# Gancheekim/ATM-VFI

Measured on AMD Instinct MI355X. Metric: interpolated frames/s at 1080p (network_base, bs=1), higher is better.
Workload: dtype f32 (contractions as fp16 hi/lo split x3 MFMA, fp32 accumulate; ~22 significand bits)

## Files before the change

### atm-vfi_amd/csrc/gemm_common.h

```cpp
#pragma once
#include "common.h"

namespace atmvfi {

struct GemmDev {
    int mode;
    const float* in;
    int in_ld, H, W, Cin;
    long long in_gstride;
    int in_rpg;
    const float* weight;
    int wrows;
    int ktot;
    int cin_pad;
    int cpt;
    int nchunks;
    int Cout;
    int coutp;
    int kw, stride, pad, dil;
    int Ho, Wo;
    long long M;
    float* out;
    int out_ld;
    long long out_gstride;
    int out_rpg;
    const int* out_row_map;
    const float* bias;
    const float* prelu;
    const float* in_prelu;
    const float* residual;
    int res_ld;
    const _Float16* w_hi;
    const _Float16* w_lo;
    int cin_pad32;
    int cpt32;
    int nchunks32;
    int ktot32;
    const _Float16* a_hi;
    const _Float16* a_lo;
    const _Float16* a_hi2;
    const _Float16* a_lo2;
    int in_ld2, split_chunks;
    int in_N;
    unsigned long long* stamp;
    int dbg;
    int mchunk;
    int vblocks;
    int nblocks;
    _Float16* out_hi;
    _Float16* out_lo;
    long long out_plane_rows;
    int out_c0, out_gc;
    int force_wn;
    int ksplit;
    float* part;
    long long part_stride;
    int part_ld;
    int fit32;
    int pfit32;
};


__device__ __forceinline__ bool gemm_out_row(const GemmDev& a, long long m, float*& orow, const float*& rrow, long long& prow, int& pc0) {
    pc0 = a.out_c0;
    if (a.mode == ATMVFI_GEMM_DECONV) {
        const int hw = a.H * a.W;
        const int n = (m >> 31) ? (int)(m / hw) : (int)((unsigned)m / (unsigned)hw);
        const int rem = (int)(m - (long long)n * hw);
        const int y = rem / a.W;
        const int x = rem - y * a.W;
        prow = ((long long)n * a.Ho + 2 * y) * a.Wo + 2 * x;
        orow = a.out + prow * a.out_ld;
    } else {
        long long ro = m;
        if (a.out_row_map) ro = a.out_row_map[m];
        if (ro < 0) return false;
        prow = ro;
        long long off = ro * (long long)a.out_ld;
        if (a.out_rpg > 0) {
            const long long grp = ro / a.out_rpg;
            prow = ro - grp * a.out_rpg;
            off = grp * a.out_gstride + prow * (long long)a.out_ld;
            pc0 += (int)grp * a.out_gc;
        }
        orow = a.out + off;
    }
    rrow = a.residual ? a.residual + m * (long long)a.res_ld : nullptr;
    return true;
}
__device__ __forceinline__ void gemm_out_row_at(const GemmDev& a, long long m, long long ro, float*& orow, long long& prow, int& pc0) {
    pc0 = a.out_c0;
    if (a.mode == ATMVFI_GEMM_DECONV) {
        const int hw = a.H * a.W;
        const int n = (m >> 31) ? (int)(m / hw) : (int)((unsigned)m / (unsigned)hw);
        const int rem = (int)(m - (long long)n * hw);
        const int y = rem / a.W;
        const int x = rem - y * a.W;
        prow = ((long long)n * a.Ho + 2 * y) * a.Wo + 2 * x;
        orow = a.out + prow * a.out_ld;
    } else {
        prow = ro;
        long long off = ro * (long long)a.out_ld;
        if (a.out_rpg > 0) {
            const long long grp = ro / a.out_rpg;
            prow = ro - grp * a.out_rpg;
            off = grp * a.out_gstride + prow * (long long)a.out_ld;
            pc0 += (int)grp * a.out_gc;
        }
        orow = a.out + off;
    }
}
__device__ __forceinline__ bool gemm_out_row(const GemmDev& a, long long m, float*& orow, const float*& rrow) {
    long long prow;
    int pc0;
    return gemm_out_row(a, m, orow, rrow, prow, pc0);
}

struct ChanVec {
    f32x4 b, p;
    int co;
    int q;
    int nvalid;
};

__device__ __forceinline__ ChanVec gemm_chan_vec(const GemmDev& a, int nb) {
    ChanVec c;
    c.q = 0;
    c.co = nb;
    if (a.mode == ATMVFI_GEMM_DECONV) {
        c.q = (nb >= a.coutp) + (nb >= 2 * a.coutp) + (nb >= 3 * a.coutp);
        c.co = nb - c.q * a.coutp;
        if (nb >= 4 * a.coutp) c.co = -1;
    }
    if (c.co >= a.Cout) c.co = -1;
    c.nvalid = c.co < 0 ? 0 : a.Cout - c.co;
    c.b = (f32x4){0.f, 0.f, 0.f, 0.f};
    c.p = (f32x4){1.f, 1.f, 1.f, 1.f};
    if (c.nvalid >= 4) {
        if (a.bias) c.b = *reinterpret_cast<const f32x4*>(a.bias + c.co);
        if (a.prelu) c.p = *reinterpret_cast<const f32x4*>(a.prelu + c.co);
    } else if (c.nvalid > 0) {
        float bb[4] = {0.f, 0.f, 0.f, 0.f}, pp[4] = {1.f, 1.f, 1.f, 1.f};
// ... 108 lines not shown
```

### atm-vfi_amd/csrc/gemm_conv.hip

```cpp
#include "common.h"
#include "gemm_common.h"

#include <algorithm>

namespace {

using atmvfi::GemmDev;

__device__ __forceinline__ int swz(int row) { return (0x1320 >> (((row >> 2) & 3) << 2)) & 3; }

template <int WM, int WN>
__global__ __launch_bounds__(256) void gemm_mfma_f32(const GemmDev a) {
    fp16_saturate_on();
    constexpr int BM = 64 * WM;
    constexpr int BN = 16 * WN;
    constexpr int NB = (BN * 4 + 255) / 256;
    __shared__ __attribute__((aligned(16))) float lds[2 * (BM + BN) * 16];
    float* As = lds;
    float* Bs = lds + 2 * BM * 16;

    const int t = threadIdx.x;
    const int lane = t & 63;
    const int wave = t >> 6;
    const int kq = t & 3;
// ... 230 lines not shown
                           "gemm: a second plane source needs CONV mode, both planes, in_ld2 > N*H*W and 0 < 32 * in_split_chunks < Cin");
        }
    }
    ATMVFI_REQUIRE(p->mode >= 0 && p->mode <= 2, ATMVFI_EINVAL, "gemm: bad mode %d", p->mode);
    ATMVFI_REQUIRE(p->Cin > 0 && p->Cout > 0, ATMVFI_EINVAL, "gemm: bad channel counts");
    ATMVFI_REQUIRE(planes || (p->in_ld >= atmvfi::round_up(p->Cin, 4) && p->in_ld % 4 == 0), ATMVFI_EALIGN,
                   "gemm: in_ld %d must be a multiple of 4 and >= Cin rounded to 4 (Cin %d)", p->in_ld, p->Cin);
    ATMVFI_REQUIRE(!p->out || (p->out_ld % 4 == 0 && p->out_ld >= atmvfi::round_up(p->Cout, 4)), ATMVFI_EALIGN,
                   "gemm: out_ld %d must be a multiple of 4 and >= Cout rounded to 4 (Cout %d)", p->out_ld, p->Cout);
    ATMVFI_REQUIRE((planes || atmvfi::aligned16(p->in)) && (!p->out || atmvfi::aligned16(p->out)) && atmvfi::aligned16(p->weight), ATMVFI_EALIGN,
                   "gemm: in/out/weight must be 16-byte aligned");
    ATMVFI_REQUIRE((planes || p->in_gstride % 4 == 0) && p->out_gstride % 4 == 0, ATMVFI_EALIGN, "gemm: group strides must be multiples of 4");
    if (p->residual)
        ATMVFI_REQUIRE(p->res_ld >= p->Cout, ATMVFI_EINVAL, "gemm: res_ld %d < Cout %d", p->res_ld, p->Cout);
    if (p->in_prelu) ATMVFI_REQUIRE(atmvfi::aligned16(p->in_prelu), ATMVFI_EALIGN, "gemm: in_prelu must be 16-byte aligned");
    ATMVFI_REQUIRE((!p->bias || atmvfi::aligned16(p->bias)) && (!p->prelu || atmvfi::aligned16(p->prelu)) &&
                       (!p->residual || (atmvfi::aligned16(p->residual) && p->res_ld % 4 == 0)),
                   ATMVFI_EALIGN, "gemm: bias/prelu/residual must be 16-byte aligned (res_ld a multiple of 4)");

    GemmDev d;
    d.mode = p->mode;
    d.in = p->in; d.in_ld = p->in_ld; d.H = p->H; d.W = p->W; d.Cin = p->Cin;
    d.in_gstride = p->in_gstride; d.in_rpg = p->in_rpg;
    d.weight = p->weight;
    d.cin_pad = atmvfi::round_up(p->Cin, 16);
    d.cpt = d.cin_pad / 16;
    d.Cout = p->Cout; d.coutp = atmvfi::round_up(p->Cout, 4);
    d.kw = 1; d.stride = 1; d.pad = 0; d.dil = 1; d.Ho = p->Ho; d.Wo = p->Wo;
    int taps = 1;
    int ngemm = p->Cout;
    if (p->mode == ATMVFI_GEMM_CONV) {
        ATMVFI_REQUIRE(p->N > 0 && p->H > 0 && p->W > 0, ATMVFI_EINVAL, "conv2d: bad input size");
        ATMVFI_REQUIRE((p->kh == 1 || p->kh == 3) && p->kh == p->kw, ATMVFI_EINVAL, "conv2d: kernel %dx%d unsupported", p->kh, p->kw);
        ATMVFI_REQUIRE(p->stride >= 1 && p->dil >= 1 && p->pad >= 0, ATMVFI_EINVAL, "conv2d: bad stride/dilation/pad");
        const int ho = (p->H + 2 * p->pad - p->dil * (p->kh - 1) - 1) / p->stride + 1;
        const int wo = (p->W + 2 * p->pad - p->dil * (p->kw - 1) - 1) / p->stride + 1;
        ATMVFI_REQUIRE(ho == p->Ho && wo == p->Wo, ATMVFI_EINVAL, "conv2d: Ho/Wo (%d,%d) do not match geometry (%d,%d)", p->Ho, p->Wo, ho, wo);
        ATMVFI_REQUIRE(p->in_rpg == 0 && p->out_rpg == 0 && !p->out_row_map, ATMVFI_EINVAL, "conv2d: row groups/maps are LINEAR-only");
        taps = p->kh * p->kw;
        d.kw = p->kw; d.stride = p->stride; d.pad = p->pad; d.dil = p->dil;
        d.M = (long long)p->N * p->Ho * p->Wo;
        ATMVFI_REQUIRE(p->M == 0 || p->M == d.M, ATMVFI_EINVAL, "conv2d: M mismatch");
    } else if (p->mode == ATMVFI_GEMM_LINEAR) {
        ATMVFI_REQUIRE(p->M > 0, ATMVFI_EINVAL, "linear: M must be > 0");
        d.H = 1; d.W = 1;
        d.M = p->M;
    } else {
        ATMVFI_REQUIRE(p->N > 0 && p->H > 0 && p->W > 0, ATMVFI_EINVAL, "deconv: bad input size");
        ATMVFI_REQUIRE(p->Ho == 2 * p->H && p->Wo == 2 * p->W, ATMVFI_EINVAL, "deconv: Ho/Wo must be 2H/2W");
        ATMVFI_REQUIRE(p->in_rpg == 0 && p->out_rpg == 0 && !p->out_row_map && !p->residual, ATMVFI_EINVAL, "deconv: unsupported option");
        d.M = (long long)p->N * p->H * p->W;
        ngemm = 4 * d.coutp;
    }
    d.wrows = packed_rows(p->mode, p->Cout);
    d.ktot = taps * d.cin_pad;
    d.nchunks = taps * d.cpt;
    d.out = p->out; d.out_ld = p->out_ld; d.out_gstride = p->out_gstride; d.out_rpg = p->out_rpg;
    d.out_row_map = p->out_row_map;
    d.bias = p->bias; d.prelu = p->prelu; d.in_prelu = p->in_prelu; d.residual = p->residual; d.res_ld = p->res_ld;
    ATMVFI_REQUIRE(d.M < (1ll << 40), ATMVFI_EINVAL, "gemm: M too large");
    d.a_hi = (const _Float16*)p->in_hi;
    d.a_lo = (const _Float16*)p->in_lo;
    d.a_hi2 = (const _Float16*)p->in_hi2;
    d.a_lo2 = (const _Float16*)p->in_lo2;
    d.in_ld2 = p->in_ld2;
    d.split_chunks = p->in_hi2 ? p->in_split_chunks : (1 << 30);
    d.in_N = p->N;
    d.out_hi = (_Float16*)p->out_hi;
    d.out_lo = (_Float16*)p->out_lo;
    d.out_plane_rows = p->out_plane_rows;
    d.out_c0 = p->out_plane_c0;
    d.out_gc = p->out_plane_gc;
    ATMVFI_REQUIRE(p->tile_wn >= -4 && p->tile_wn <= 8 && (p->tile_wn >= 0 || planes), ATMVFI_EINVAL,
                   "gemm: tile_wn 0 (auto), 1..8, or (split-plane input) -1 reference schedule / -2 gemm_duo (128-column tiles) / -3 gemm_pp / -4 gemm_duo (64-column tiles), got %d", p->tile_wn);
    d.force_wn = p->tile_wn;
    ATMVFI_REQUIRE(!p->workspace || (atmvfi::aligned16(p->workspace) && p->workspace_floats > 0), ATMVFI_EALIGN,
                   "gemm: the split-K workspace must be 16-byte aligned and non-empty");
    d.ksplit = 0;
    d.part = p->workspace;
    d.part_stride = p->workspace ? p->workspace_floats : 0;
    d.part_ld = 0;
    d.fit32 = 0;
    d.pfit32 = 0;
    d.nblocks = 0;
    d.dbg = 0;
    d.vblocks = 0;
    d.mchunk = 0;
    d.stamp = nullptr;
    d.w_hi = (const _Float16*)p->weight_hi;
    d.w_lo = (const _Float16*)p->weight_lo;
    d.cin_pad32 = atmvfi::round_up(p->Cin, 32);
    d.cpt32 = d.cin_pad32 / 32;
    d.nchunks32 = taps * d.cpt32;
    d.ktot32 = taps * d.cin_pad32;
    if (p->precision == ATMVFI_PREC_F16X3) {
        ATMVFI_REQUIRE(p->weight_hi && p->weight_lo, ATMVFI_EINVAL, "gemm: precision f16x3 needs weight_hi/weight_lo");
        ATMVFI_REQUIRE(atmvfi::aligned16(p->weight_hi) && atmvfi::aligned16(p->weight_lo), ATMVFI_EALIGN,
                       "gemm: split weights must be 16-byte aligned");
        if (planes) return atmvfi::launch_gemm_split(d, ngemm, (hipStream_t)stream);
        return atmvfi::launch_gemm_f16x3(d, ngemm, (hipStream_t)stream);
    }

    {
        int rc = 0;
        if (atmvfi::try_launch_conv3x3_small(d, p->kh, &rc, (hipStream_t)stream)) return rc;
    }
    const int ntiles = (ngemm + 15) / 16;
    int best = 1;
    float best_cost = 1e30f;
    for (int wn = 1; wn <= 8; ++wn) {
        const int padded = (ntiles + wn - 1) / wn * wn;
        const float cost = (float)padded * (1.0f + 1.0f / (float)wn);
        if (cost <= best_cost) { best_cost = cost; best = wn; }
    }
    hipStream_t s = (hipStream_t)stream;
    switch (best) {
        case 1: launch<2, 1>(d, ntiles, s); break;
        case 2: launch<2, 2>(d, ntiles, s); break;
        case 3: launch<2, 3>(d, ntiles, s); break;
        case 4: launch<2, 4>(d, ntiles, s); break;
        case 5: launch<2, 5>(d, ntiles, s); break;
        case 6: launch<2, 6>(d, ntiles, s); break;
        case 7: launch<2, 7>(d, ntiles, s); break;
        default: launch<2, 8>(d, ntiles, s); break;
    }
    return atmvfi::check_launch("gemm");
}

extern "C" int atmvfi_conv2d(const atmvfi_gemm_params* p, void* stream) {
    ATMVFI_REQUIRE(p && p->mode == ATMVFI_GEMM_CONV, ATMVFI_EINVAL, "conv2d: params->mode must be ATMVFI_GEMM_CONV");
    return atmvfi_gemm(p, stream);
}
extern "C" int atmvfi_linear(const atmvfi_gemm_params* p, void* stream) {
    ATMVFI_REQUIRE(p && p->mode == ATMVFI_GEMM_LINEAR, ATMVFI_EINVAL, "linear: params->mode must be ATMVFI_GEMM_LINEAR");
    return atmvfi_gemm(p, stream);
}
extern "C" int atmvfi_deconv2x2(const atmvfi_gemm_params* p, void* stream) {
    ATMVFI_REQUIRE(p && p->mode == ATMVFI_GEMM_DECONV, ATMVFI_EINVAL, "deconv2x2: params->mode must be ATMVFI_GEMM_DECONV");
    return atmvfi_gemm(p, stream);
}
```

### atm-vfi_amd/csrc/gemm_duo.hip

```cpp
#include "gemm_plane.h"

namespace {

using atmvfi::GemmDev;

constexpr int BM = 128;
constexpr int stage_bytes(int BN) { return (2 * BM + 2 * BN) * 64; }
constexpr int A_LO = BM * 64, W_HI = 2 * BM * 64;
constexpr int cst_floats(int BN) { return atmvfi::gemm_const_floats(BN) + BM; }

#ifdef ATMVFI_STAMP
static unsigned long long* g_duo_stamp = nullptr;
extern "C" void atmvfi_debug_set_duo_stamp_buffer(void* p) { g_duo_stamp = (unsigned long long*)p; }
#define DUO_SUB(k) do { if (a.stamp) { __builtin_amdgcn_sched_barrier(0); const unsigned long long t_ = __builtin_amdgcn_s_memtime(); sub[k] += t_ - sub_t; sub_t = t_; __builtin_amdgcn_sched_barrier(0); } } while (0)
#else
#define DUO_SUB(k) do { } while (0)
#endif

template <bool CONVM, int BN>
__global__ __launch_bounds__(256, 2) void gemm_duo_kernel(const GemmDev a) {
    constexpr int STAGE = stage_bytes(BN), W_LO = W_HI + BN * 64;
    constexpr int MI = BN == 128 ? 4 : 2;
    constexpr int NWN = BN / 64;
    constexpr int WROWS = 16 * MI;
// ... 71 lines not shown
            dma16(pa_lo + aoff[1], dst + A_LO + 4 * 1024);
            pa_hi += a_step;
            pa_lo += a_step;
        }
        dma16(pw_hi + wsoff[0], dst + W_HI);
        if constexpr (PIW == 2) dma16(pw_hi + wsoff[1], dst + W_HI + 4 * 1024);
        dma16(pw_lo + wsoff[0], dst + W_LO);
        if constexpr (PIW == 2) dma16(pw_lo + wsoff[1], dst + W_LO + 4 * 1024);
        pw_hi += w_step;
        pw_lo += w_step;
    };
    {
        atmvfi::gemm_dma_consts<BN>(a, n0, cst_w, wave, lane);
        if (a.out_row_map && a.mode == ATMVFI_GEMM_LINEAR) {
            int m = m0 + (wave & 1) * 64 + lane;
            if (m >= M) m = M - 1;
            __builtin_amdgcn_global_load_lds((const __attribute__((address_space(1))) void*)(a.out_row_map + m),
                                             (__attribute__((address_space(3))) void*)(cst_w + atmvfi::gemm_const_floats(BN) + (wave & 1) * 64), 4, 0, 0);
        } else {
            atmvfi::gemm_dma_consts<BN>(a, n0, cst_w, wave, lane);
        }
    }

    f32x4 acc[MI][4], cor[MI][4];
#pragma unroll
    for (int i = 0; i < MI; ++i)
#pragma unroll
        for (int j = 0; j < 4; ++j) {
            acc[i][j] = (f32x4){0.f, 0.f, 0.f, 0.f};
            cor[i][j] = (f32x4){0.f, 0.f, 0.f, 0.f};
        }
#ifdef ATMVFI_STAMP
    unsigned long long sub[8] = {0, 0, 0, 0, 0, 0, 0, 0}, sub_t = 0, t_begin = 0;
    if (a.stamp) { t_begin = sub_t = __builtin_amdgcn_s_memtime(); }
#endif
    issue_stage(0);
    if (nk > 1) issue_stage(1);
    DUO_SUB(0);
    f16x8 xh[MI], xl[MI], wh[4], wl[4];
    const unsigned xfrag = lds_offset(smem) + (unsigned)((WROWS * wm + r) * 64 + ((g ^ swz64(r)) << 4));
    const unsigned wfrag = lds_offset(smem) + (unsigned)(W_HI + (64 * wn + r) * 64 + ((g ^ swz64(r)) << 4));
    for (int u = 0; u < nk; ++u) {
        if (u + 1 < nk) wait_vm<4 + 2 * PIW>();
        else wait_vm<0>();
        __builtin_amdgcn_s_barrier();
        DUO_SUB(1);
        const unsigned off = (unsigned)((u & 1) * STAGE);
        static_for<0, MI>([&](auto ic) {
            constexpr int i = decltype(ic)::value;
            lds_read16<i * 1024>(xh[i], xfrag + off);
            lds_read16<i * 1024 + A_LO>(xl[i], xfrag + off);
        });
        static_for<0, 4>([&](auto jc) {
            constexpr int j = decltype(jc)::value;
            lds_read16<j * 1024>(wh[j], wfrag + off);
            lds_read16<j * 1024 + BN * 64>(wl[j], wfrag + off);
        });
        asm volatile("s_waitcnt lgkmcnt(0)" : "+v"(xh[0]), "+v"(xh[1]), "+v"(xl[0]), "+v"(xl[1]));
        if constexpr (MI == 4) asm volatile("" : "+v"(xh[2]), "+v"(xh[3]), "+v"(xl[2]), "+v"(xl[3]));
#pragma unroll
        for (int j = 0; j < 4; ++j) asm volatile("" : "+v"(wh[j]), "+v"(wl[j]));
        DUO_SUB(2);
        __builtin_amdgcn_s_barrier();
        DUO_SUB(3);
        if (u + 2 < nk) issue_stage(u & 1);
        DUO_SUB(4);
        __builtin_amdgcn_s_setprio(1);
#pragma unroll
        for (int i = 0; i < MI; ++i)
#pragma unroll
            for (int j = 0; j < 4; ++j) {
                cor[i][j] = __builtin_amdgcn_mfma_f32_16x16x32_f16(wl[j], xh[i], cor[i][j], 0, 0, 0);
                acc[i][j] = __builtin_amdgcn_mfma_f32_16x16x32_f16(wh[j], xh[i], acc[i][j], 0, 0, 0);
            }
#pragma unroll
        for (int i = 0; i < MI; ++i)
#pragma unroll
            for (int j = 0; j < 4; ++j) cor[i][j] = __builtin_amdgcn_mfma_f32_16x16x32_f16(wh[j], xl[i], cor[i][j], 0, 0, 0);
        __builtin_amdgcn_s_setprio(0);
        DUO_SUB(5);
    }
    {
        __builtin_amdgcn_s_barrier();
#pragma unroll
        for (int i = 0; i < MI; ++i)
#pragma unroll
            for (int j = 0; j < 4; ++j) {
                acc[i][j] = acc[i][j] + cor[i][j] * LO_UNSCALE;
                asm volatile("" : "+v"(acc[i][j]));
            }
        {
            const unsigned tb = lds_offset(smem) + (unsigned)(wave * 4096);
            const unsigned wbase = tb + (unsigned)(r * 256);
            const unsigned rbase = tb + (unsigned)(g * 256);
            unsigned wad[4], rad[4];
#pragma unroll
            for (int k = 0; k < 4; ++k) {
                wad[k] = wbase + (unsigned)((((4 * k + g) ^ r) & 15) << 4);
                rad[k] = rbase + (unsigned)(k * 1024) + (unsigned)(((r ^ (4 * k + g)) & 15) << 4);
            }
            static_for<0, MI>([&](auto ic) {
                constexpr int i = decltype(ic)::value;
                static_for<0, 4>([&](auto jc) {
                    constexpr int j = decltype(jc)::value;
                    lds_write16f(wad[j], acc[i][j]);
                });
                static_for<0, 4>([&](auto qc) {
                    constexpr int q = decltype(qc)::value;
                    lds_read16f<0>(acc[i][q], rad[q]);
                });
            });
            asm volatile("s_waitcnt lgkmcnt(0)" ::: "memory");
#pragma unroll
            for (int i = 0; i < MI; ++i)
#pragma unroll
                for (int q = 0; q < 4; ++q) asm volatile("" : "+v"(acc[i][q]));
        }
        if (a.ksplit > 1) {
            float* pb = a.part + blockIdx.y * a.part_stride + (n0 + 64 * wn + 4 * r);
#pragma unroll
            for (int i = 0; i < MI; ++i)
#pragma unroll
                for (int q = 0; q < 4; ++q) {
                    const int m = m0 + WROWS * wm + g + 16 * i + 4 * q;
                    if (m < M) *reinterpret_cast<f32x4*>(pb + (long long)m * a.part_ld) = acc[i][q];
                }
            return;
        }
        atmvfi::plane_gemm_epilogue<CONVM, MI, BM, BN>(a, acc, cst, m0, n0, M, wm, wn, r, g);
    }
#ifdef ATMVFI_STAMP
    DUO_SUB(6);
    if (a.stamp && lane == 0) {
        unsigned long long* o = a.stamp + ((long long)blockIdx.x * 4 + wave) * 8;
        for (int k = 0; k < 7; ++k) o[k] = sub[k];
        o[7] = sub_t - t_begin;
    }
#endif
}

__global__ __launch_bounds__(256) void gemm_splitk_reduce_kernel(const GemmDev a, int ngemm4) {
    fp16_saturate_on();
    const long long total = a.M * (long long)ngemm4;
    for (long long idx = (long long)blockIdx.x * blockDim.x + threadIdx.x; idx < total; idx += (long long)gridDim.x * blockDim.x) {
        const long long m = idx / ngemm4;
        const int nb = (int)(idx - m * ngemm4) * 4;
        const atmvfi::ChanPos cp = atmvfi::gemm_chan_pos(a, nb);
        if (cp.nvalid <= 0) continue;
        auto vec4 = [&](const float* t, float dflt) -> f32x4 {
            if (!t) return (f32x4){dflt, dflt, dflt, dflt};
            if (cp.nvalid >= 4) return *reinterpret_cast<const f32x4*>(t + cp.co);
            f32x4 o = (f32x4){t[cp.co], dflt, dflt, dflt};
            if (cp.nvalid > 1) o.y = t[cp.co + 1];
            if (cp.nvalid > 2) o.z = t[cp.co + 2];
            return o;
        };
        const float* p = a.part + m * a.part_ld + nb;
        f32x4 v = *reinterpret_cast<const f32x4*>(p);
        for (int sp = 1; sp < a.ksplit; ++sp) v += *reinterpret_cast<const f32x4*>(p + sp * a.part_stride);
        float* orow;
        const float* rrow;
        long long prow;
        int pc0;
        if (!atmvfi::gemm_out_row(a, m, orow, rrow, prow, pc0)) continue;
        const f32x4 res = rrow ? atmvfi::gemm_load_residual4(rrow, cp) : (f32x4){0.f, 0.f, 0.f, 0.f};
        atmvfi::gemm_finish_store4(a, orow, prow, pc0, cp, v, vec4(a.bias, 0.f), vec4(a.prelu, 1.f), res);
    }
}

}

template <bool CONVM, int BN>
static int launch_duo(const GemmDev& d, int ngemm, hipStream_t s) {
    const size_t lds = (size_t)2 * stage_bytes(BN) + cst_floats(BN) * sizeof(float);
    const hipError_t attr_err = atmvfi::allow_dynamic_lds<gemm_duo_kernel<CONVM, BN>>(lds);
    ATMVFI_REQUIRE(attr_err == hipSuccess, ATMVFI_ELAUNCH, "gemm_duo: hipFuncSetAttribute: %s", hipGetErrorString(attr_err));
    GemmDev dd = d;
    const int prc = atmvfi::plane_gemm_prepare("gemm_duo", dd, ngemm, BM, BN);
    if (prc != ATMVFI_OK) return prc;
#ifdef ATMVFI_STAMP
    dd.stamp = g_duo_stamp;
#endif
    if (dd.ksplit > 1) {
        hipLaunchKernelGGL((gemm_duo_kernel<CONVM, BN>), dim3((unsigned)dd.vblocks, (unsigned)dd.ksplit), dim3(256), lds, s, dd);
        const int rc = atmvfi::check_launch("gemm_duo (split-K)");
        if (rc != ATMVFI_OK) return rc;
        const int ngemm4 = (ngemm + 3) / 4;
        const long long groups = d.M * ngemm4;
        hipLaunchKernelGGL(gemm_splitk_reduce_kernel, dim3((unsigned)std::min<long long>((groups + 255) / 256, 8192)), dim3(256), 0, s, dd, ngemm4);
        return atmvfi::check_launch("gemm_duo (split-K reduce)");
    }
    hipLaunchKernelGGL((gemm_duo_kernel<CONVM, BN>), dim3((unsigned)dd.vblocks), dim3(256), lds, s, dd);
    return atmvfi::check_launch("gemm_duo");
}

int atmvfi::launch_gemm_duo(const GemmDev& d, int ngemm, hipStream_t s) {
    if ((ngemm <= 64 && d.force_wn != -2) || d.force_wn == -4)
        return d.mode == ATMVFI_GEMM_CONV ? launch_duo<true, 64>(d, ngemm, s) : launch_duo<false, 64>(d, ngemm, s);
    return d.mode == ATMVFI_GEMM_CONV ? launch_duo<true, 128>(d, ngemm, s) : launch_duo<false, 128>(d, ngemm, s);
}
```

### atm-vfi_amd/csrc/gemm_plane.h

```cpp
#pragma once
#include "common.h"
#include "gemm_common.h"

typedef _Float16 f16x8 __attribute__((ext_vector_type(8)));

constexpr float LO_UNSCALE = 1.0f / 1024.0f;

__device__ __forceinline__ int swz64(int row) { return ((row >> 2) & 1) << 1; }
__device__ __forceinline__ void dma16(const unsigned char* src, unsigned char* lds_wave_base) {
    __builtin_amdgcn_global_load_lds((const __attribute__((address_space(1))) void*)src,
                                     (__attribute__((address_space(3))) void*)lds_wave_base, 16, 0, 0);
}
__device__ __forceinline__ void lds_write16f(unsigned addr, const f32x4& v) {
    asm volatile("ds_write_b128 %0, %1" ::"v"(addr), "v"(v) : "memory");
}
template <int OFF>
__device__ __forceinline__ void lds_read16f(f32x4& d, unsigned addr) {
    asm volatile("ds_read_b128 %0, %1 offset:%2" : "=v"(d) : "v"(addr), "n"(OFF) : "memory");
}
template <int N>
__device__ __forceinline__ void wait_vm() { asm volatile("s_waitcnt vmcnt(%0)" ::"n"(N) : "memory"); }

namespace atmvfi {

// ... 218 lines not shown
                    for (int q = 0; q < 4; ++q) {
                        const f32x4 v = finish(i, q);
                        const unsigned rr = ro[i][q] < 0 ? 0u : (unsigned)ro[i][q];
                        const unsigned gi = rr / rpg;
                        const long long prow = rr - gi * rpg;
                        if (ro[i][q] >= 0 && col_ok) {
                            if constexpr (F32) *reinterpret_cast<f32x4*>(a.out + gi * a.out_gstride + prow * (long long)a.out_ld + nb) = v;
                            sink_store4(sink, prow, a.out_c0 + (int)gi * a.out_gc + nb, v);
                        }
                    }
            };
            if (a.out_rpg == 0 && a.pfit32) {
                if (a.out) rows32(std::true_type{});
                else rows32(std::false_type{});
            } else if (a.out) rows(std::true_type{});
            else rows(std::false_type{});
        } else {
            const RowSink sink{nullptr, 0, a.out_hi, a.out_lo, a.out_plane_rows};
            const int hw = a.H * a.W;
            int dn = (int)((unsigned)mrow / (unsigned)hw);
            const int rem = mrow - dn * hw;
            int dy = rem / a.W;
            int dx = rem - dy * a.W;
            const int qoff = (cp.q >> 1) * a.Wo + (cp.q & 1);
            const int pc = a.out_c0 + cp.co;
            if (a.pfit32) {
                const long long cpart = ((long long)(pc >> 5) * a.out_plane_rows) * 32 + (pc & 31);
                unsigned char* ph = reinterpret_cast<unsigned char*>(a.out_hi + cpart);
                unsigned char* pl = reinterpret_cast<unsigned char*>(a.out_lo + cpart);
                unsigned rowbase = ((unsigned)dn * (unsigned)a.Ho + 2u * (unsigned)dy) * (unsigned)a.Wo + (unsigned)qoff;
                const unsigned rstep = 2u * (unsigned)a.Wo;
#pragma unroll
                for (int i = 0; i < MI; ++i)
#pragma unroll
                    for (int q = 0; q < 4; ++q) {
                        const f32x4 v = finish(i, q, false);
                        const unsigned boff = (rowbase + 2u * (unsigned)dx) << 6;
                        if (ro[i][q] >= 0 && cp.nvalid > 0) {
                            f16x2 h0, l0, h1, l1;
                            split_pair((f32x2){v.x, v.y}, h0, l0);
                            split_pair((f32x2){v.z, v.w}, h1, l1);
                            *reinterpret_cast<f16x4*>(ph + boff) = (f16x4){h0.x, h0.y, h1.x, h1.y};
                            *reinterpret_cast<f16x4*>(pl + boff) = (f16x4){l0.x, l0.y, l1.x, l1.y};
                        }
                        dx += 4;
                        const bool wrap = dx >= a.W;
                        dx = wrap ? dx - a.W : dx;
                        rowbase += wrap ? rstep : 0u;
                    }
            } else
#pragma unroll
            for (int i = 0; i < MI; ++i)
#pragma unroll
                for (int q = 0; q < 4; ++q) {
                    f32x4 v = finish(i, q);
                    v.y = cp.nvalid > 1 ? v.y : 0.f;
                    v.z = cp.nvalid > 2 ? v.z : 0.f;
                    v.w = cp.nvalid > 3 ? v.w : 0.f;
                    const long long prow = ((long long)dn * a.Ho + 2 * dy) * a.Wo + 2 * dx + qoff;
                    if (ro[i][q] >= 0 && cp.nvalid > 0) sink_store4(sink, prow, pc, v);
                    dx += 4;
                    const bool wrap = dx >= a.W;
                    dx = wrap ? dx - a.W : dx;
                    dy = wrap ? dy + 1 : dy;
                    const bool wrap2 = dy >= a.H;
                    dy = wrap2 ? 0 : dy;
                    dn = wrap2 ? dn + 1 : dn;
                }
        }
    };
    const bool c4 = (a.Cout & 3) == 0;
    const bool fast = (a.mode != ATMVFI_GEMM_DECONV && c4 && (a.out_hi || (a.out && a.out_rpg == 0))) ||
                      (a.mode == ATMVFI_GEMM_DECONV && !a.out && a.out_hi && a.W >= 4 && !a.residual);
    if (fast) {
        if (a.prelu) fast_rows(std::true_type{});
        else fast_rows(std::false_type{});
    } else if (a.residual && !vec_res) {
        store_rows(std::true_type{});
    } else {
        store_rows(std::false_type{});
    }
}

inline int plane_gemm_prepare(const char* engine, GemmDev& d, int ngemm, int BM, int BN) {
    ATMVFI_REQUIRE((long long)d.in_ld * 64 < (1ll << 32) && (long long)d.wrows * 64 < (1ll << 32) &&
                       (!d.a_hi2 || (long long)d.in_ld2 * 64 < (1ll << 32)) && d.M < (1ll << 26), ATMVFI_EINVAL,
                   "%s: plane rows x 64 bytes must fit 32 bits (got %d rows)", engine, d.in_ld);
    if (d.mode == ATMVFI_GEMM_CONV)
        ATMVFI_REQUIRE(d.H < 32768 && d.W < 32768, ATMVFI_EINVAL, "%s: CONV mode packs (y, x) into 16 bits each", engine);
    d.dbg = 0;
    d.pfit32 = d.out_hi && (long long)d.out_plane_rows * 64 < (1ll << 32);
    d.fit32 = d.out && !d.out_row_map && d.out_rpg == 0 && d.mode != ATMVFI_GEMM_DECONV && (d.M + 1) * (long long)d.out_ld * 4 < (1ll << 32) &&
               (!d.residual || (d.M + 1) * (long long)d.res_ld * 4 < (1ll << 32));
    d.nblocks = (ngemm + BN - 1) / BN;
    const long long mgroups = (ceil_div64(d.M, BM) + 7) / 8;
    ATMVFI_REQUIRE(mgroups * 8 * d.nblocks < (1LL << 31), ATMVFI_EINVAL, "%s: grid too large", engine);
    d.vblocks = (int)(mgroups * 8 * d.nblocks);
    return ATMVFI_OK;
}

}
```

### atm-vfi_amd/csrc/gemm_pp.hip

```cpp
#include "gemm_plane.h"

#ifdef ATMVFI_STAMP
static unsigned long long* g_pp_stamp = nullptr;
extern "C" void atmvfi_debug_set_pp_stamp_buffer(void* p) { g_pp_stamp = (unsigned long long*)p; }
#define PP_KSTAMP_BEGIN() unsigned long long kt0_ = 0; do { if (a.stamp) { __builtin_amdgcn_sched_barrier(0); kt0_ = __builtin_amdgcn_s_memtime(); __builtin_amdgcn_sched_barrier(0); } } while (0)
#define PP_KSTAMP_END(idx) do { if (a.stamp) { __builtin_amdgcn_sched_barrier(0); const unsigned long long t_ = __builtin_amdgcn_s_memtime(); if (lane == 0) atomicAdd(&kst[wave * 16 + ((idx) < 15 ? (idx) : 15)], t_ - kt0_); __builtin_amdgcn_sched_barrier(0); } } while (0)
#define PP_STAMP(i) do { if (a.stamp) { tstamp[i] = __builtin_amdgcn_s_memtime(); rstamp[i] = __builtin_amdgcn_s_memrealtime(); } } while (0)
#define PP_SUB(k) do { if (a.stamp) { __builtin_amdgcn_sched_barrier(0); const unsigned long long t_ = __builtin_amdgcn_s_memtime(); sub[k] += t_ - sub_t; sub_t = t_; __builtin_amdgcn_sched_barrier(0); } } while (0)
#else
#define PP_STAMP(i) do { } while (0)
#define PP_SUB(k) do { } while (0)
#define PP_KSTAMP_BEGIN() do { } while (0)
#define PP_KSTAMP_END(idx) do { } while (0)
#endif

namespace {

using atmvfi::GemmDev;

constexpr int BM = 256, BN = 128;
constexpr int STAGE = (2 * BM + 2 * BN) * 64;
constexpr int A_LO = BM * 64, W_HI = 2 * BM * 64, W_LO = W_HI + BN * 64;
constexpr int PIECES = 6;
constexpr int CST_FLOATS = atmvfi::gemm_const_floats(BN) + BM;
// ... 152 lines not shown
                else wait_vm<0>();
            } else {
                if (has_next) wait_vm<PIECES>();
            }
        };
        if (grp == 1 && g1wait) wait_next();
        asm volatile("s_waitcnt lgkmcnt(0)"
                     : "+v"(xh[0]), "+v"(xh[1]), "+v"(xh[2]), "+v"(xh[3]), "+v"(xl[0]), "+v"(xl[1]), "+v"(xl[2]), "+v"(xl[3]));
#pragma unroll
        for (int j = 0; j < 4; ++j) asm volatile("" : "+v"(wh[j]), "+v"(wl[j]));
        __builtin_amdgcn_sched_barrier(0);
        __builtin_amdgcn_s_barrier();
        __builtin_amdgcn_sched_barrier(0);
        __builtin_amdgcn_s_setprio(1);
#pragma unroll
        for (int i = 0; i < 4; ++i)
#pragma unroll
            for (int j = 0; j < 4; ++j) {
                cor[i][j] = __builtin_amdgcn_mfma_f32_16x16x32_f16(wl[j], xh[i], cor[i][j], 0, 0, 0);
                acc[i][j] = __builtin_amdgcn_mfma_f32_16x16x32_f16(wh[j], xh[i], acc[i][j], 0, 0, 0);
            }
#pragma unroll
        for (int i = 0; i < 4; ++i)
#pragma unroll
            for (int j = 0; j < 4; ++j) cor[i][j] = __builtin_amdgcn_mfma_f32_16x16x32_f16(wh[j], xl[i], cor[i][j], 0, 0, 0);
        __builtin_amdgcn_s_setprio(0);
        if (grp == 0) wait_next();
        __builtin_amdgcn_sched_barrier(0);
        __builtin_amdgcn_s_barrier();
        __builtin_amdgcn_sched_barrier(0);
    };

    for (;;) {
        const int nxt = vb + grid;
        has_next = false;
        if (nxt < a.vblocks) {
            tile_of(nxt, nm0, nn0);
            has_next = nm0 < M;
        }
        const float* cst = cst_base + (seq & 1) * CST_FLOATS;
#pragma unroll
        for (int i = 0; i < 4; ++i)
#pragma unroll
            for (int j = 0; j < 4; ++j) {
                acc[i][j] = (f32x4){0.f, 0.f, 0.f, 0.f};
                cor[i][j] = (f32x4){0.f, 0.f, 0.f, 0.f};
                asm volatile("" : "+v"(acc[i][j]), "+v"(cor[i][j]));
            }
        PP_STAMP(1);
        {
            bool g1wait = seq == 0;
            for (int kc = 0; kc + 2 < nk; ++kc) {
                PP_KSTAMP_BEGIN();
                kstep(std::integral_constant<int, 0>{}, g1wait);
                PP_KSTAMP_END(kc);
                g1wait = true;
            }
            if (nk >= 2) {
                PP_KSTAMP_BEGIN();
                kstep(std::integral_constant<int, 1>{}, g1wait);
                PP_KSTAMP_END(nk - 2);
                g1wait = true;
            }
            {
                PP_KSTAMP_BEGIN();
                kstep(std::integral_constant<int, 2>{}, g1wait);
                PP_KSTAMP_END(nk - 1);
            }
        }
        PP_STAMP(2);
#ifdef ATMVFI_STAMP
        sub_t = __builtin_amdgcn_s_memtime();
#endif
        if (grp == 0) __builtin_amdgcn_s_barrier();
        if (grp == 1 && has_next) wait_vm<0>();

#pragma unroll
        for (int i = 0; i < 4; ++i)
#pragma unroll
            for (int j = 0; j < 4; ++j) {
                acc[i][j] = acc[i][j] + cor[i][j] * LO_UNSCALE;
                asm volatile("" : "+v"(acc[i][j]));
            }
        {
            const unsigned xb = (unsigned)(rd_off == 0 ? 2 * STAGE : rd_off - STAGE);
            const unsigned tb = lds_offset(smem) + xb + (unsigned)(wave * 1024);
            const unsigned wbase = tb + (unsigned)((r >> 2) * 8192 + (r & 3) * 256 + ((g ^ (r & 3)) << 4));
            const unsigned rq6 = (unsigned)((r >> 2) << 6);
            const unsigned rbase = tb + (unsigned)(g * 256);
            const unsigned rg4 = (unsigned)((r ^ g) << 4);
            unsigned wad[4], rad[4];
#pragma unroll
            for (int k = 0; k < 4; ++k) {
                wad[k] = wbase + (rq6 ^ (unsigned)(k << 6));
                rad[k] = rbase + (rg4 ^ (unsigned)(k << 6));
            }
            static_for<0, 4>([&](auto ic) {
                constexpr int i = decltype(ic)::value;
                static_for<0, 4>([&](auto jc) {
                    constexpr int j = decltype(jc)::value;
                    lds_write16f(wad[j], acc[i][j]);
                });
                static_for<0, 4>([&](auto qc) {
                    constexpr int q = decltype(qc)::value;
                    lds_read16f<q * 8192>(acc[i][q], rad[q]);
                });
            });
            asm volatile("s_waitcnt lgkmcnt(0)" ::: "memory");
#pragma unroll
            for (int i = 0; i < 4; ++i)
#pragma unroll
                for (int q = 0; q < 4; ++q) asm volatile("" : "+v"(acc[i][q]));
        }
        PP_SUB(0);
        atmvfi::plane_gemm_epilogue<CONVM, 4, BM, BN>(a, acc, cst, m0, n0, M, wm, wn, r, g, [&] { PP_SUB(1); });
        PP_SUB(2);
        PP_STAMP(3);
#ifdef ATMVFI_STAMP
        if (a.stamp) {
            if (seq == 0) { t_pro = tstamp[1] - tstamp[0]; r_pro = rstamp[1] - rstamp[0]; }
            t_loop += tstamp[2] - tstamp[1]; r_loop += rstamp[2] - rstamp[1];
            t_epi += tstamp[3] - tstamp[2]; r_epi += rstamp[3] - rstamp[2];
            ++ntile;
        }
#endif
        if (!has_next) break;
        if (grp == 1) __builtin_amdgcn_s_barrier();
        vb = nxt;
        m0 = nm0;
        n0 = nn0;
        ++seq;
    }
#ifdef ATMVFI_STAMP
    if (a.stamp && lane == 0) {
        unsigned long long* o = a.stamp + ((long long)blockIdx.x * 8 + wave) * 8;
        o[0] = t_pro; o[1] = t_loop / ntile; o[2] = t_epi / ntile;
        o[3] = (unsigned long long)nk;
        o[4] = r_loop / ntile; o[5] = sub[0] / ntile; o[6] = sub[1] / ntile;
        o[7] = sub[2] / ntile;
    }
    __syncthreads();
    if (a.stamp && tid < 128) a.stamp[(long long)gridDim.x * 64 + (long long)blockIdx.x * 128 + tid] = kst[tid] / (ntile ? ntile : 1);
#endif
}

}

template <bool CONVM>
static int launch_pp(const GemmDev& d, int ngemm, hipStream_t s) {
#ifdef ATMVFI_STAMP
    const size_t lds = (size_t)3 * STAGE + 2 * CST_FLOATS * sizeof(float) + 1024;
#else
    const size_t lds = (size_t)3 * STAGE + 2 * CST_FLOATS * sizeof(float);
#endif
    const hipError_t attr_err = atmvfi::allow_dynamic_lds<gemm_pp_kernel<CONVM>>(lds);
    ATMVFI_REQUIRE(attr_err == hipSuccess, ATMVFI_ELAUNCH, "gemm_pp: hipFuncSetAttribute: %s", hipGetErrorString(attr_err));
    GemmDev dd = d;
    const int rc = atmvfi::plane_gemm_prepare("gemm_pp", dd, ngemm, BM, BN);
    if (rc != ATMVFI_OK) return rc;
#ifdef ATMVFI_STAMP
    dd.stamp = g_pp_stamp;
#endif
    const int grid = d.nchunks32 >= 2 ? std::min(dd.vblocks, atmvfi::cu_count()) : dd.vblocks;
    hipLaunchKernelGGL(gemm_pp_kernel<CONVM>, dim3((unsigned)grid), dim3(512), lds, s, dd);
    return atmvfi::check_launch("gemm_pp");
}

int atmvfi::launch_gemm_pp(const GemmDev& d, int ngemm, hipStream_t s) {
    return d.mode == ATMVFI_GEMM_CONV ? launch_pp<true>(d, ngemm, s) : launch_pp<false>(d, ngemm, s);
}
```

Measured before the change: 51.13.

## Add 16-byte fp16 plane store epilogue with remapped LDS transpose for full tiles

```diff
diff --git a/atm-vfi_amd/csrc/gemm_common.h b/atm-vfi_amd/csrc/gemm_common.h
--- a/atm-vfi_amd/csrc/gemm_common.h
+++ b/atm-vfi_amd/csrc/gemm_common.h
@@ -58,6 +58,7 @@
     int part_ld;
     int fit32;
     int pfit32;
+    int sink16;
 };
 
 
diff --git a/atm-vfi_amd/csrc/gemm_conv.hip b/atm-vfi_amd/csrc/gemm_conv.hip
--- a/atm-vfi_amd/csrc/gemm_conv.hip
+++ b/atm-vfi_amd/csrc/gemm_conv.hip
@@ -336,6 +336,7 @@
     d.part_ld = 0;
     d.fit32 = 0;
     d.pfit32 = 0;
+    d.sink16 = 0;
     d.nblocks = 0;
     d.dbg = 0;
     d.vblocks = 0;
diff --git a/atm-vfi_amd/csrc/gemm_duo.hip b/atm-vfi_amd/csrc/gemm_duo.hip
--- a/atm-vfi_amd/csrc/gemm_duo.hip
+++ b/atm-vfi_amd/csrc/gemm_duo.hip
@@ -177,6 +177,9 @@
     }
     {
         __builtin_amdgcn_s_barrier();
+        const bool sink16 = a.sink16 && m0 + BM <= M;
+        int r16 = r, g16 = g;
+        asm volatile("" : "+v"(r16), "+v"(g16));
 #pragma unroll
         for (int i = 0; i < MI; ++i)
 #pragma unroll
@@ -193,6 +196,13 @@
             for (int k = 0; k < 4; ++k) {
                 wad[k] = wbase + (unsigned)((((4 * k + g) ^ r) & 15) << 4);
                 rad[k] = rbase + (unsigned)(k * 1024) + (unsigned)(((r ^ (4 * k + g)) & 15) << 4);
+            }
+            if (sink16) {
+#pragma unroll
+                for (int k = 0; k < 4; ++k) {
+                    const int R = atmvfi::plane_sink16_read_row(r16, g16, k >> 1);
+                    rad[k] = tb + (unsigned)(R * 256) + (unsigned)((((2 * (r16 & 7) + (k & 1)) ^ R) & 15) << 4);
+                }
             }
             static_for<0, MI>([&](auto ic) {
                 constexpr int i = decltype(ic)::value;
@@ -222,7 +232,8 @@
                 }
             return;
         }
-        atmvfi::plane_gemm_epilogue<CONVM, MI, BM, BN>(a, acc, cst, m0, n0, M, wm, wn, r, g);
+        if (sink16) atmvfi::plane_gemm_epilogue_sink16<CONVM, MI, BN>(a, acc, cst, m0, n0, wm, wn, r16, g16);
+        else atmvfi::plane_gemm_epilogue<CONVM, MI, BM, BN>(a, acc, cst, m0, n0, M, wm, wn, r, g);
     }
 #ifdef ATMVFI_STAMP
     DUO_SUB(6);
diff --git a/atm-vfi_amd/csrc/gemm_plane.h b/atm-vfi_amd/csrc/gemm_plane.h
--- a/atm-vfi_amd/csrc/gemm_plane.h
+++ b/atm-vfi_amd/csrc/gemm_plane.h
@@ -324,6 +324,101 @@
     }
 }
 
+__device__ __forceinline__ int plane_sink16_read_row(int r, int g, int h) { return 8 * h + 2 * g + (r >> 3); }
+template <bool CONVM, int MI, int BN, typename Hook = NoHook>
+__device__ __forceinline__ void plane_gemm_epilogue_sink16(const GemmDev a, f32x4 (&acc)[MI][4], const float* cst, int m0, int n0, int wm, int wn,
+                                                           int r, int g, Hook after_residuals = Hook{}) {
+    typedef unsigned u32x4 __attribute__((ext_vector_type(4)));
+    constexpr int WROWS = 16 * MI;
+    const int cl = 64 * wn + 8 * (r & 7);
+    const int nb = n0 + cl;
+    const f32x4 b0 = *reinterpret_cast<const f32x4*>(cst + cl), b1 = *reinterpret_cast<const f32x4*>(cst + cl + 4);
+    const f32x4 p0 = *reinterpret_cast<const f32x4*>(cst + BN + cl), p1 = *reinterpret_cast<const f32x4*>(cst + BN + cl + 4);
+    const int mrow = m0 + WROWS * wm + 2 * g + (r >> 3);
+    const float sv = cst[BN + 64 * wn + 16 * g + r];
+    const bool pmax = __builtin_amdgcn_ballot_w64(!(sv >= 0.f && sv <= 1.f)) == 0ull;
+    after_residuals();
+    auto rows = [&](auto act_tag, auto kind_tag) {
+        constexpr int ACT = decltype(act_tag)::value;
+        constexpr int KIND = decltype(kind_tag)::value;
+        auto finish = [&](const f32x4 x, const f32x4& b, const f32x4& p) -> f32x4 {
+            f32x4 v = x + b;
+            if constexpr (ACT == 1) {
+                v.x = v.x > 0.f ? v.x : p.x * v.x;
+                v.y = v.y > 0.f ? v.y : p.y * v.y;
+                v.z = v.z > 0.f ? v.z : p.z * v.z;
+                v.w = v.w > 0.f ? v.w : p.w * v.w;
+            } else if constexpr (ACT == 2) {
+                const f32x4 t = p * v;
+                f32x4 o;
+                asm("v_max_f32 %0, %1, %2" : "=v"(o.x) : "v"(v.x), "v"(t.x));
+                asm("v_max_f32 %0, %1, %2" : "=v"(o.y) : "v"(v.y), "v"(t.y));
+                asm("v_max_f32 %0, %1, %2" : "=v"(o.z) : "v"(v.z), "v"(t.z));
+                asm("v_max_f32 %0, %1, %2" : "=v"(o.w) : "v"(v.w), "v"(t.w));
+                v = o;
+            }
+            return v;
+        };
+        auto bits = [](f16x2 v) { return __builtin_bit_cast(unsigned, v); };
+        int c = a.out_c0 + nb;
+        bool col_ok = nb < a.Cout;
+        unsigned x = 0, qoff = 0;
+        if constexpr (KIND == 2) {
+            const ChanPos cp = gemm_chan_pos(a, nb);
+            c = a.out_c0 + cp.co;
+            col_ok = cp.nvalid > 0;
+            x = (unsigned)mrow % (unsigned)a.W;
+            qoff = (unsigned)((cp.q >> 1) * a.Wo + (cp.q & 1));
+        }
+        if (!col_ok) return;
+        const long long cpart = ((long long)(c >> 5) * a.out_plane_rows) * 32 + (c & 31);
+        unsigned char* ph = reinterpret_cast<unsigned char*>(a.out_hi + cpart);
+        unsigned char* pl = reinterpret_cast<unsigned char*>(a.out_lo + cpart);
+        const unsigned w = (unsigned)a.W;
+        const unsigned base = KIND == 2 ? 4u * (unsigned)mrow + qoff : (unsigned)mrow;
+#pragma unroll
+        for (int i = 0; i < MI; ++i)
+#pragma unroll
+            for (int h = 0; h < 2; ++h) {
+                const f32x4 v0 = finish(acc[i][2 * h], b0, p0), v1 = finish(acc[i][2 * h + 1], b1, p1);
+                constexpr unsigned ROWSTEP = KIND == 2 ? 4u : 1u;
+                unsigned prow = base + ROWSTEP * (unsigned)(16 * i + 8 * h);
+                if constexpr (KIND == 2) prow -= 2u * x;
+                if constexpr (KIND == 1) {
+                    float* o = a.out + (unsigned long long)prow * (unsigned)a.out_ld + nb;
+                    *reinterpret_cast<f32x4*>(o) = v0;
+                    *reinterpret_cast<f32x4*>(o + 4) = v1;
+                }
+                f16x2 h0, l0, h1, l1, h2, l2, h3, l3;
+                split_pair((f32x2){v0.x, v0.y}, h0, l0);
+                split_pair((f32x2){v0.z, v0.w}, h1, l1);
+                split_pair((f32x2){v1.x, v1.y}, h2, l2);
+                split_pair((f32x2){v1.z, v1.w}, h3, l3);
+                const unsigned boff = prow << 6;
+                *reinterpret_cast<u32x4*>(ph + boff) = (u32x4){bits(h0), bits(h1), bits(h2), bits(h3)};
+                *reinterpret_cast<u32x4*>(pl + boff) = (u32x4){bits(l0), bits(l1), bits(l2), bits(l3)};
+                if constexpr (KIND == 2) {
+                    x += 8u;
+                    x = min(x, x - w);
+                    x = min(x, x - w);
+                }
+            }
+    };
+    auto kinds = [&](auto act_tag) {
+        if constexpr (!CONVM) {
+            if (a.mode == ATMVFI_GEMM_DECONV) {
+                rows(act_tag, std::integral_constant<int, 2>{});
+                return;
+            }
+        }
+        if (a.out) rows(act_tag, std::integral_constant<int, 1>{});
+        else rows(act_tag, std::integral_constant<int, 0>{});
+    };
+    if (!a.prelu) kinds(std::integral_constant<int, 0>{});
+    else if (pmax) kinds(std::integral_constant<int, 2>{});
+    else kinds(std::integral_constant<int, 1>{});
+}
+
 inline int plane_gemm_prepare(const char* engine, GemmDev& d, int ngemm, int BM, int BN) {
     ATMVFI_REQUIRE((long long)d.in_ld * 64 < (1ll << 32) && (long long)d.wrows * 64 < (1ll << 32) &&
                        (!d.a_hi2 || (long long)d.in_ld2 * 64 < (1ll << 32)) && d.M < (1ll << 26), ATMVFI_EINVAL,
@@ -334,6 +429,8 @@
     d.pfit32 = d.out_hi && (long long)d.out_plane_rows * 64 < (1ll << 32);
     d.fit32 = d.out && !d.out_row_map && d.out_rpg == 0 && d.mode != ATMVFI_GEMM_DECONV && (d.M + 1) * (long long)d.out_ld * 4 < (1ll << 32) &&
                (!d.residual || (d.M + 1) * (long long)d.res_ld * 4 < (1ll << 32));
+    d.sink16 = d.pfit32 && (d.out_c0 & 7) == 0 && !d.residual && !d.out_row_map && d.out_rpg == 0 && d.ksplit <= 1 &&
+               (d.mode == ATMVFI_GEMM_DECONV ? !d.out && d.W >= 4 && (d.coutp & 7) == 0 : (d.Cout & 7) == 0);
     d.nblocks = (ngemm + BN - 1) / BN;
     const long long mgroups = (ceil_div64(d.M, BM) + 7) / 8;
     ATMVFI_REQUIRE(mgroups * 8 * d.nblocks < (1LL << 31), ATMVFI_EINVAL, "%s: grid too large", engine);
diff --git a/atm-vfi_amd/csrc/gemm_pp.hip b/atm-vfi_amd/csrc/gemm_pp.hip
--- a/atm-vfi_amd/csrc/gemm_pp.hip
+++ b/atm-vfi_amd/csrc/gemm_pp.hip
@@ -258,6 +258,8 @@
                 acc[i][j] = acc[i][j] + cor[i][j] * LO_UNSCALE;
                 asm volatile("" : "+v"(acc[i][j]));
             }
+        const bool sink16 = a.sink16 && m0 + BM <= M;
+        int r16 = r, g16 = g;
         {
             const unsigned xb = (unsigned)(rd_off == 0 ? 2 * STAGE : rd_off - STAGE);
             const unsigned tb = lds_offset(smem) + xb + (unsigned)(wave * 1024);
@@ -269,7 +271,15 @@
 #pragma unroll
             for (int k = 0; k < 4; ++k) {
                 wad[k] = wbase + (rq6 ^ (unsigned)(k << 6));
-                rad[k] = rbase + (rg4 ^ (unsigned)(k << 6));
+                rad[k] = rbase + (rg4 ^ (unsigned)(k << 6)) + (unsigned)(k * 8192);
+            }
+            if (sink16) {
+                asm volatile("" : "+v"(r16), "+v"(g16));
+#pragma unroll
+                for (int k = 0; k < 4; ++k) {
+                    const int R = atmvfi::plane_sink16_read_row(r16, g16, k >> 1);
+                    rad[k] = tb + (unsigned)((R >> 2) * 8192 + (R & 3) * 256) + (unsigned)((((2 * (r16 & 7) + (k & 1)) ^ R) & 15) << 4);
+                }
             }
             static_for<0, 4>([&](auto ic) {
                 constexpr int i = decltype(ic)::value;
@@ -279,7 +289,7 @@
                 });
                 static_for<0, 4>([&](auto qc) {
                     constexpr int q = decltype(qc)::value;
-                    lds_read16f<q * 8192>(acc[i][q], rad[q]);
+                    lds_read16f<0>(acc[i][q], rad[q]);
                 });
             });
             asm volatile("s_waitcnt lgkmcnt(0)" ::: "memory");
@@ -289,7 +299,8 @@
                 for (int q = 0; q < 4; ++q) asm volatile("" : "+v"(acc[i][q]));
         }
         PP_SUB(0);
-        atmvfi::plane_gemm_epilogue<CONVM, 4, BM, BN>(a, acc, cst, m0, n0, M, wm, wn, r, g, [&] { PP_SUB(1); });
+        if (sink16) atmvfi::plane_gemm_epilogue_sink16<CONVM, 4, BN>(a, acc, cst, m0, n0, wm, wn, r16, g16, [&] { PP_SUB(1); });
+        else atmvfi::plane_gemm_epilogue<CONVM, 4, BM, BN>(a, acc, cst, m0, n0, M, wm, wn, r, g, [&] { PP_SUB(1); });
         PP_SUB(2);
         PP_STAMP(3);
 #ifdef ATMVFI_STAMP
```

Result: no change. 51.24 (median of 6 runs) (+0.2%).
